# UzL-ITS/dash

Measured on AMD Instinct MI355X. Metric: online garbled inferences/sec (MiniONN CIFAR-10 CNN), higher is better.
Workload: dtype uint8 label components / int8 MFMA (exact modular arithmetic)

## Files before the change

### dash_amd/csrc/hip/mrs_chain.h

```cpp
#pragma once

#include "gadget_common.h"

namespace dash {
namespace dev {

__device__ __forceinline__ u128 add_packed(u128 a, u128 b, u128 hmask) {
    return ((a & ~hmask) + (b & ~hmask)) ^ ((a ^ b) & hmask);
}

#ifndef DASH_MRS_CHUNK
#define DASH_MRS_CHUNK 4
#endif
constexpr int kMrsChunk = DASH_MRS_CHUNK;
#ifndef DASH_MRS_M2CH
#define DASH_MRS_M2CH 16
#endif
template <int K>
__device__ __forceinline__ constexpr int mrs_pair(int l, int j) {
    return l * (2 * K - l - 1) / 2 + (j - l - 1);
}

template <int MODE>
__device__ __forceinline__ constexpr uint32_t mrs_row_sub(int i) {
    return tw_sub(MODE == 1 ? kTwSmrs : kTwMrs, static_cast<uint32_t>(i));
}
__device__ __forceinline__ void store_ypads(const MrsArgs& a, u128 key, int b, int64_t N, int64_t e) {
    const uint64_t g = a.rgate0 ^ static_cast<uint64_t>(e);
    for (int blk = 0; 4 * blk < a.ny; ++blk) {
        u128 p[4];
        hard_block(key, g, tw_sub(kTwMmy, 0), static_cast<uint32_t>(blk), p);
#pragma unroll
        for (int q = 0; q < 4; ++q)
            if (4 * blk + q < a.ny) a.ys[(static_cast<int64_t>(b) * a.ny + 4 * blk + q) * N + e] = p[q];
    }
}

template <int MODE>
__device__ __forceinline__ void store_sign_key(const MrsArgs& a, u128 key, int b, int64_t N, int64_t e) {
    if (MODE >= 1 && a.ks) a.ks[static_cast<int64_t>(b) * N + e] = key;
}

#ifndef DASH_CHAIN2_WAVES
#define DASH_CHAIN2_WAVES 4
#endif
template <int K, int MODE>
__global__ __launch_bounds__(kAesBlock, MODE == 2 ? DASH_CHAIN2_WAVES : DASH_UA_MINBLOCKS) void k_mrs_chain(MrsArgs a, Act x, const ModC* mc,
                                                                          const uint32_t* te0, const uint32_t* rk) {
    (void)te0;
    (void)rk;
    const int b = blockIdx.z;
    const int64_t N = a.N;
    constexpr int NP = K * (K - 1) / 2 > 0 ? K * (K - 1) / 2 : 1;
    for (int64_t e = static_cast<int64_t>(blockIdx.x) * blockDim.x + threadIdx.x; e < N;
         e += static_cast<int64_t>(gridDim.x) * blockDim.x) {
        const u128* row0 = a.tab + (static_cast<int64_t>(b) * N + e) * a.n_tab;
        u128* PS = a.ps + static_cast<int64_t>(b) * NP * N + e;
        u128 acc = 0;
#pragma unroll
        for (int i = 0; i < (MODE >= 1 ? K - 1 : K); ++i) {
            const int r = MODE >= 1 ? (i + 1) % K : i;
            const ModC m = mc[a.crt.p[r]];
            const int n = static_cast<int>(m.n);
            const act_t* L = x.p[r] + static_cast<int64_t>(b) * n * N + e;
            DigitStream ds[K > 1 ? K - 1 : 1];
#pragma unroll
            for (int l = 0; l < i; ++l) ds[l].init(PS[static_cast<int64_t>(mrs_pair<K>(l, i)) * N]);
            CompressFwd cf;
            cf.init();
            uint32_t col = 0;
            uint16_t cur[kMrsChunk], nxt[kMrsChunk];
#pragma unroll
            for (int u = 0; u < kMrsChunk; ++u)
                if (u < n) cur[u] = static_cast<uint16_t>(L[static_cast<int64_t>(u) * N]);
            for (int c0 = 0; c0 < n; c0 += kMrsChunk) {
#pragma unroll
                for (int u = 0; u < kMrsChunk; ++u)
                    if (c0 + kMrsChunk + u < n) nxt[u] = static_cast<uint16_t>(L[static_cast<int64_t>(c0 + kMrsChunk + u) * N]);
#pragma unroll
                for (int u = 0; u < kMrsChunk; ++u)
                    if (c0 + u < n) {
                        uint32_t d = cur[u];
#pragma unroll
                        for (int l = 0; l < i; ++l) {
                            const uint32_t s = ds[l].next(m);
                            d = d >= s ? d - s : d + m.q - s;
                        }
                        if (c0 + u == 0) col = d;
                        cf.push(d, m);
                    }
#pragma unroll
                for (int u = 0; u < kMrsChunk; ++u) cur[u] = nxt[u];
            }
            constexpr int kExtra = MODE == 1 ? 0 : 1;
            const int nt = K - 1 - i + kExtra;
            const u128* row = row0 + a.dig_off[i] + static_cast<int64_t>(col) * nt;
            u128 E[K];
#pragma unroll
            for (int t = 0; t < nt; ++t) E[t] = row[t];
            hard_unmask_n<K>(E, nt, cf.finish(), a.gate0 ^ static_cast<uint64_t>(e), mrs_row_sub<MODE>(i));
#pragma unroll
            for (int t = 0; t < K - 1 - i; ++t) PS[static_cast<int64_t>(mrs_pair<K>(i, i + 1 + t)) * N] = E[t];
            if (MODE != 1) acc = add_packed(acc, E[K - 1 - i], a.hmask);
        }
        if (MODE >= 1) {
            const ModC m = mc[a.crt.p[0]];
            const act_t* L = x.p[0] + static_cast<int64_t>(b) * m.n * N + e;
            u128 key = compress_cm<DASH_MRS_M2CH>(L, N, m);
#pragma unroll
            for (int l = 0; l < K - 1; ++l) key ^= PS[static_cast<int64_t>(mrs_pair<K>(l, K - 1)) * N];
            const uint32_t c = static_cast<uint32_t>(key) & 1u;
            u128 E = 0;
            if (MODE == 2)
                E = row0[a.dig_off[K - 1] + c] - hard_pad(key, a.gate0 ^ static_cast<uint64_t>(e), mrs_row_sub<MODE>(K - 1), 0);
            store_ypads(a, key, b, N, e);
            store_sign_key<MODE>(a, key, b, N, e);
            a.cs[static_cast<int64_t>(b) * N + e] = static_cast<uint8_t>(c);
            if (MODE == 2) acc = add_packed(acc, E, a.hmask);
        }
        if (MODE == 1) continue;
        const uint32_t col = static_cast<uint32_t>(acc) & static_cast<uint32_t>(a.T - 1);
        const u128* row = row0 + a.fin_off + static_cast<int64_t>(col) * K;
        u128 F[K];
#pragma unroll
        for (int j = 0; j < K; ++j) F[j] = row[j];
        hard_unmask<K>(F, acc, a.gate0 ^ static_cast<uint64_t>(e), mrs_row_sub<0>(K));
#pragma unroll
        for (int j = 0; j < K; ++j) a.pf[(static_cast<int64_t>(b) * K + j) * N + e] = F[j];
    }
}

constexpr int kMrsBS = 512;
constexpr int kMrsCap = 64;
#ifndef DASH_STAGE_U
#define DASH_STAGE_U 2
#endif
constexpr int kStageU = DASH_STAGE_U;
#ifndef DASH_STAGE_RD
#define DASH_STAGE_RD 4
#endif
constexpr int kStageRd = DASH_STAGE_RD;
template <int K, int MODE, int I>
__device__ __forceinline__ void chain_s_pos(const MrsArgs& a, uint64_t gate, const ModC* mc, const Act& x,
                                            uint8_t* stg, int b, int64_t N, int64_t e0, int tid, bool valid,
                                            const u128* row0, u128* PS, u128& acc) {
    constexpr int kLast = MODE >= 1 ? K - 1 : K;
    if constexpr (I < kLast) {
        constexpr int i = I;
        {
            constexpr int r = MODE >= 1 ? (i + 1) % K : i;
            const ModC m = mc[a.crt.p[r]];
            const int n = static_cast<int>(m.n);
            const act_t* L = x.p[r] + static_cast<int64_t>(b) * n * N;
            uint32_t col = 0;
            u128 key;
            constexpr int kExtra = MODE == 1 ? 0 : 1;
            constexpr int nt = K - 1 - i + kExtra;
            u128 pf0 = 0, pf1 = 0;
            if constexpr (r == 0) {
                DigitStream ds[K > 1 ? K - 1 : 1];
#pragma unroll
                for (int l = 0; l < i; ++l) ds[l].init(PS[static_cast<int64_t>(mrs_pair<K>(l, i)) * N]);
                CompressFwd cf;
                cf.init();
                for (int c0 = 0; c0 < n; c0 += kMrsCap) {
                    const int cnt = min(kMrsCap, n - c0);
                    __syncthreads();
                    lds_stage_rows<kMrsBS, kStageU>(stg, L, N, e0, c0, cnt);
                    __syncthreads();
                    for (int c = 0; c < cnt; ++c) {
                        uint32_t d = valid ? stg[c * kMrsBS + tid] : 0u;
#pragma unroll
                        for (int l = 0; l < i; ++l) {
                            const uint32_t s = ds[l].next(m);
                            d = d >= s ? d - s : d + m.q - s;
                        }
                        if (c0 + c == 0) {
                            col = d;
                            const u128* rowp = row0 + a.dig_off[i] + static_cast<int64_t>(col) * nt;
                            pf0 = rowp[0];
                            pf1 = rowp[nt - 1];
                        }
                        cf.push(d, m);
                    }
                }
                key = cf.finish();
            } else {
                u128 Q[K > 1 ? K - 1 : 1];
#pragma unroll
                for (int l = 0; l < i; ++l) Q[l] = PS[static_cast<int64_t>(mrs_pair<K>(l, i)) * N];
                u128 C = 0, PW = 1;
                const int mcn = static_cast<int>(m.c);
                const int pass = kMrsCap / mcn * mcn;
                for (int p0 = 0; p0 < n; p0 += pass) {
                    const int pcnt = min(pass, n - p0);
                    __syncthreads();
                    lds_stage_rows<kMrsBS, kStageU>(stg, L, N, e0, p0, pcnt);
                    __syncthreads();
                    for (int c0 = 0; c0 < pcnt; c0 += mcn) {
                        uint32_t rr[K > 1 ? K - 1 : 1];
#pragma unroll
                        for (int l = 0; l < i; ++l) rr[l] = divmod128(Q[l], m);
                        const int cnt = min(mcn, pcnt - c0);
                        uint32_t v = 0, pt = 1;
                        auto digit = [&](int t) -> uint32_t {
                            uint32_t d = valid ? stg[(c0 + t) * kMrsBS + tid] : 0u;
#pragma unroll
                            for (int l = 0; l < i; ++l) {
                                const uint32_t sd = chunk_digit(rr[l], m);
                                d = d >= sd ? d - sd : d + m.q - sd;
                            }
                            return d;
                        };
                        int t0 = 0;
                        if (p0 + c0 == 0) {
                            const uint32_t d = digit(0);
                            col = d;
                            const u128* rowp = row0 + a.dig_off[i] + static_cast<int64_t>(col) * nt;
                            pf0 = rowp[0];
                            pf1 = rowp[nt - 1];
                            v = d;
                            pt = m.q;
                            t0 = 1;
                        }
#pragma unroll 2
                        for (int t = t0; t < cnt; ++t) {
                            const uint32_t d = digit(t);
                            v += d * pt;
                            pt *= m.q;
                        }
                        C += PW * static_cast<u128>(v);
                        PW *= static_cast<u128>(m.D);
                    }
                }
                key = C;
            }
            const u128* row = row0 + a.dig_off[i] + static_cast<int64_t>(col) * nt;
            u128 E[K];
            E[0] = pf0;
#pragma unroll
            for (int t = 1; t < nt - 1; ++t) E[t] = row[t];
            if (nt > 1) E[nt - 1] = pf1;
            hard_unmask_n<K>(E, nt, key, gate, mrs_row_sub<MODE>(i));
            if (valid) {
#pragma unroll
                for (int t = 0; t < K - 1 - i; ++t) PS[static_cast<int64_t>(mrs_pair<K>(i, i + 1 + t)) * N] = E[t];
            }
            if constexpr (MODE != 1) acc = add_packed(acc, E[K - 1 - i], a.hmask);
        }
        chain_s_pos<K, MODE, I + 1>(a, gate, mc, x, stg, b, N, e0, tid, valid, row0, PS, acc);
    }
}

template <int K, int MODE>
__global__ __launch_bounds__(kMrsBS, MODE == 2 ? DASH_CHAIN2_WAVES : DASH_UA_MINBLOCKS) void k_mrs_chain_s(
    MrsArgs a, Act x, const ModC* mc, const uint32_t* te0, const uint32_t* rk) {
    (void)te0;
    (void)rk;
    __shared__ __attribute__((aligned(16))) uint8_t stg[kMrsCap * kMrsBS];
    const int b = blockIdx.z;
    const int64_t N = a.N;
    constexpr int NP = K * (K - 1) / 2 > 0 ? K * (K - 1) / 2 : 1;
    const int tid = static_cast<int>(threadIdx.x);
    for (int64_t e0 = static_cast<int64_t>(blockIdx.x) * kMrsBS; e0 < N; e0 += static_cast<int64_t>(gridDim.x) * kMrsBS) {
        const bool valid = e0 + tid < N;
        const int64_t e = valid ? e0 + tid : N - 1;
        const u128* row0 = a.tab + (static_cast<int64_t>(b) * N + e) * a.n_tab;
        u128* PS = a.ps + static_cast<int64_t>(b) * NP * N + e;
        u128 acc = 0;
        const uint64_t gate = a.gate0 ^ static_cast<uint64_t>(e);
        chain_s_pos<K, MODE, 0>(a, gate, mc, x, stg, b, N, e0, tid, valid, row0, PS, acc);
        if (MODE >= 1) {
            const ModC m = mc[a.crt.p[0]];
            const int n = static_cast<int>(m.n);
            const act_t* L = x.p[0] + static_cast<int64_t>(b) * n * N;
            CompressFwd cf;
            cf.init();
            u128 kb = 0;
            for (int c0 = 0; c0 < n; c0 += kMrsCap) {
                const int cnt = min(kMrsCap, n - c0);
                __syncthreads();
                lds_stage_rows<kMrsBS, kStageU>(stg, L, N, e0, c0, cnt);
                __syncthreads();
                if (m.bits == 1) {
                    for (int w0 = 0; w0 < cnt; w0 += 32) {
                        uint32_t w = 0;
#pragma unroll 8
                        for (int u = 0; u < 32; ++u)
                            if (w0 + u < cnt) w |= (valid ? static_cast<uint32_t>(stg[(w0 + u) * kMrsBS + tid]) : 0u) << u;
                        kb |= static_cast<u128>(w) << (c0 + w0);
                    }
                } else {
                    for (int c = 0; c < cnt; ++c) cf.push(valid ? stg[c * kMrsBS + tid] : 0u, m);
                }
            }
            u128 key = m.bits == 1 ? kb : cf.finish();
#pragma unroll
            for (int l = 0; l < K - 1; ++l) key ^= PS[static_cast<int64_t>(mrs_pair<K>(l, K - 1)) * N];
            const uint32_t c = static_cast<uint32_t>(key) & 1u;
            u128 E = 0;
            if (MODE == 2) E = row0[a.dig_off[K - 1] + c] - hard_pad(key, gate, mrs_row_sub<MODE>(K - 1), 0);
            if (valid) {
                store_ypads(a, key, b, N, e);
                store_sign_key<MODE>(a, key, b, N, e);
                a.cs[static_cast<int64_t>(b) * N + e] = static_cast<uint8_t>(c);
            }
            if (MODE == 2) acc = add_packed(acc, E, a.hmask);
        }
        if (MODE == 1) continue;
        const uint32_t colf = static_cast<uint32_t>(acc) & static_cast<uint32_t>(a.T - 1);
        const u128* row = row0 + a.fin_off + static_cast<int64_t>(colf) * K;
        u128 F[K];
#pragma unroll
        for (int j = 0; j < K; ++j) F[j] = row[j];
        hard_unmask<K>(F, acc, gate, mrs_row_sub<0>(K));
        if (valid) {
#pragma unroll
            for (int j = 0; j < K; ++j) a.pf[(static_cast<int64_t>(b) * K + j) * N + e] = F[j];
        }
    }
}

constexpr int kMrsWBS = 256;
constexpr int kWaveU = 8;
template <int K, int MODE, int I>
__device__ __forceinline__ void chain_w_pos(const MrsArgs& a, uint64_t gate, const ModC* mc, const uint8_t* wst,
                                            const int* roff, int tid, bool valid, const u128* row0, u128* PS,
                                            u128& acc) {
    constexpr int kLast = MODE >= 1 ? K - 1 : K;
    if constexpr (I < kLast) {
        constexpr int r = MODE >= 1 ? (I + 1) % K : I;
        const ModC m = mc[a.crt.p[r]];
        const int n = static_cast<int>(m.n);
        const uint8_t* Ls = wst + roff[r] * kMrsWBS + tid;
        uint32_t col = 0;
        u128 key;
        constexpr int kExtra = MODE == 1 ? 0 : 1;
        constexpr int nt = K - 1 - I + kExtra;
        u128 pf0 = 0, pf1 = 0;
        if constexpr (r == 0) {
            DigitStream ds[I > 0 ? I : 1];
#pragma unroll
            for (int l = 0; l < I; ++l) ds[l].init(PS[mrs_pair<K>(l, I)]);
            CompressFwd cf;
            cf.init();
            for (int c = 0; c < n; ++c) {
                uint32_t d = valid ? Ls[c * kMrsWBS] : 0u;
#pragma unroll
                for (int l = 0; l < I; ++l) {
                    const uint32_t s = ds[l].next(m);
                    d = d >= s ? d - s : d + m.q - s;
                }
                if (c == 0) {
                    col = d;
                    const u128* rowp = row0 + a.dig_off[I] + static_cast<int64_t>(col) * nt;
                    pf0 = rowp[0];
                    pf1 = rowp[nt - 1];
                }
                cf.push(d, m);
            }
            key = cf.finish();
        } else {
            u128 Q[I > 0 ? I : 1];
#pragma unroll
            for (int l = 0; l < I; ++l) Q[l] = PS[mrs_pair<K>(l, I)];
            u128 C = 0, PW = 1;
            for (int c0 = 0; c0 < n; c0 += static_cast<int>(m.c)) {
                uint32_t rr[I > 0 ? I : 1];
#pragma unroll
                for (int l = 0; l < I; ++l) rr[l] = divmod128(Q[l], m);
                const int cnt = min(static_cast<int>(m.c), n - c0);
                uint32_t v = 0, pt = 1;
                for (int t = 0; t < cnt; ++t) {
                    uint32_t d = valid ? Ls[(c0 + t) * kMrsWBS] : 0u;
#pragma unroll
                    for (int l = 0; l < I; ++l) {
                        const uint32_t sd = chunk_digit(rr[l], m);
                        d = d >= sd ? d - sd : d + m.q - sd;
                    }
                    if (c0 + t == 0) {
                        col = d;
                        const u128* rowp = row0 + a.dig_off[I] + static_cast<int64_t>(col) * nt;
                        pf0 = rowp[0];
                        pf1 = rowp[nt - 1];
                    }
                    v += d * pt;
                    pt *= m.q;
                }
                C += PW * static_cast<u128>(v);
                PW *= static_cast<u128>(m.D);
            }
            key = C;
        }
        const u128* row = row0 + a.dig_off[I] + static_cast<int64_t>(col) * nt;
        u128 E[nt > 0 ? nt : 1];
        E[0] = pf0;
#pragma unroll
        for (int t = 1; t < nt - 1; ++t) E[t] = row[t];
        if constexpr (nt > 1) E[nt - 1] = pf1;
        if constexpr (nt > 0) hard_unmask<nt>(E, key, gate, mrs_row_sub<MODE>(I));
#pragma unroll
        for (int t = 0; t < K - 1 - I; ++t) PS[mrs_pair<K>(I, I + 1 + t)] = E[t];
        if constexpr (MODE != 1) acc = add_packed(acc, E[K - 1 - I], a.hmask);
        chain_w_pos<K, MODE, I + 1>(a, gate, mc, wst, roff, tid, valid, row0, PS, acc);
    }
}

template <int K, int MODE>
__global__ __launch_bounds__(kMrsWBS, 1) void k_mrs_chain_w(MrsArgs a, Act x, const ModC* mc, const uint32_t* te0,
                                                            const uint32_t* rk) {
    (void)te0;
    (void)rk;
    extern __shared__ __attribute__((aligned(16))) uint8_t wst[];
    const int b = blockIdx.z;
    const int64_t N = a.N;
    constexpr int NP = K * (K - 1) / 2 > 0 ? K * (K - 1) / 2 : 1;
    const int tid = static_cast<int>(threadIdx.x);
    int roff[K + 1];
    const act_t* src[K];
    roff[0] = 0;
#pragma unroll
    for (int r = 0; r < K; ++r) {
        const int n = static_cast<int>(mc[a.crt.p[r]].n);
        roff[r + 1] = roff[r] + n;
        src[r] = x.p[r] + static_cast<int64_t>(b) * n * N;
    }
    const int units = roff[K] * (kMrsWBS / 16);
    for (int64_t e0 = static_cast<int64_t>(blockIdx.x) * kMrsWBS; e0 < N; e0 += static_cast<int64_t>(gridDim.x) * kMrsWBS) {
        __syncthreads();
        if (N % 16 != 0) {
            constexpr int kWaveBU = 32;
            const int bunits = roff[K] * kMrsWBS;
            const int64_t e = e0 + tid;
            for (int x0 = tid; x0 < bunits; x0 += kWaveBU * kMrsWBS) {
                uint32_t v[kWaveBU];
#pragma unroll
                for (int h = 0; h < kWaveBU; ++h) {
                    const int xu = x0 + h * kMrsWBS;
                    const int g = xu / kMrsWBS;
                    const act_t* row = src[0] + static_cast<int64_t>(g) * N;
#pragma unroll
                    for (int r = 1; r < K; ++r)
                        if (g >= roff[r]) row = src[r] + static_cast<int64_t>(g - roff[r]) * N;
                    v[h] = (xu < bunits && e < N) ? static_cast<uint32_t>(row[e]) : 0u;
                }
#pragma unroll
                for (int h = 0; h < kWaveBU; ++h) {
                    const int xu = x0 + h * kMrsWBS;
                    if (xu < bunits) wst[xu] = static_cast<uint8_t>(v[h]);
                }
            }
        } else
        for (int x0 = tid; x0 < units; x0 += kWaveU * kMrsWBS) {
            uint4 v[kWaveU];
#pragma unroll
            for (int h = 0; h < kWaveU; ++h) {
                const int xu = x0 + h * kMrsWBS;
                const int g = xu >> 4;
                const int64_t e = e0 + 16 * (xu & 15);
                const act_t* row = src[0] + static_cast<int64_t>(g) * N;
#pragma unroll
                for (int r = 1; r < K; ++r)
                    if (g >= roff[r]) row = src[r] + static_cast<int64_t>(g - roff[r]) * N;
                if (xu < units && e < N) v[h] = *reinterpret_cast<const uint4*>(row + e);
            }
#pragma unroll
            for (int h = 0; h < kWaveU; ++h) {
                const int xu = x0 + h * kMrsWBS;
                if (xu < units) *reinterpret_cast<uint4*>(wst + (xu >> 4) * kMrsWBS + 16 * (xu & 15)) = v[h];
            }
        }
        __syncthreads();
        const bool valid = e0 + tid < N;
        const int64_t e = valid ? e0 + tid : N - 1;
        const u128* row0 = a.tab + (static_cast<int64_t>(b) * N + e) * a.n_tab;
        u128 PS[NP];
        u128 acc = 0;
        const uint64_t gate = a.gate0 ^ static_cast<uint64_t>(e);
        chain_w_pos<K, MODE, 0>(a, gate, mc, wst, roff, tid, valid, row0, PS, acc);
        if (MODE >= 1) {
            const ModC m = mc[a.crt.p[0]];
            const int n = static_cast<int>(m.n);
            const uint8_t* Ls = wst + tid;
            CompressFwd cf;
            cf.init();
            for (int c = 0; c < n; ++c) cf.push(valid ? Ls[c * kMrsWBS] : 0u, m);
            u128 key = cf.finish();
#pragma unroll
            for (int l = 0; l < K - 1; ++l) key ^= PS[mrs_pair<K>(l, K - 1)];
            const uint32_t cb = static_cast<uint32_t>(key) & 1u;
            u128 E = 0;
            if (MODE == 2) E = row0[a.dig_off[K - 1] + cb] - hard_pad(key, gate, mrs_row_sub<MODE>(K - 1), 0);
            if (valid) {
                store_ypads(a, key, b, N, e);
                store_sign_key<MODE>(a, key, b, N, e);
                a.cs[static_cast<int64_t>(b) * N + e] = static_cast<uint8_t>(cb);
            }
            if (MODE == 2) acc = add_packed(acc, E, a.hmask);
        }
        if (MODE == 1) continue;
        const uint32_t colf = static_cast<uint32_t>(acc) & static_cast<uint32_t>(a.T - 1);
        const u128* row = row0 + a.fin_off + static_cast<int64_t>(colf) * K;
        u128 F[K];
#pragma unroll
        for (int j = 0; j < K; ++j) F[j] = row[j];
        hard_unmask<K>(F, acc, gate, mrs_row_sub<0>(K));
        if (valid) {
#pragma unroll
            for (int j = 0; j < K; ++j) a.pf[(static_cast<int64_t>(b) * K + j) * N + e] = F[j];
        }
    }
}

constexpr int kMrsQE = 64;
constexpr int kMrsQBS = 4 * kMrsQE;
template <int S>
__device__ __forceinline__ uint32_t quad_bcast(uint32_t v) {
    return static_cast<uint32_t>(__builtin_amdgcn_mov_dpp(static_cast<int>(v), S * 0x55, 0xF, 0xF, false));
}
template <int S>
__device__ __forceinline__ u128 quad_bcast128(u128 v) {
    const uint32_t w0 = quad_bcast<S>(static_cast<uint32_t>(v)), w1 = quad_bcast<S>(static_cast<uint32_t>(v >> 32));
    const uint32_t w2 = quad_bcast<S>(static_cast<uint32_t>(v >> 64)), w3 = quad_bcast<S>(static_cast<uint32_t>(v >> 96));
    return (static_cast<u128>((static_cast<uint64_t>(w3) << 32) | w2) << 64) | ((static_cast<uint64_t>(w1) << 32) | w0);
}
__device__ __forceinline__ uint32_t quad_sum_mod(uint32_t v, uint32_t q) {
    uint32_t s = v + static_cast<uint32_t>(__builtin_amdgcn_mov_dpp(static_cast<int>(v), 0xB1, 0xF, 0xF, false));
    s = s >= q ? s - q : s;
    uint32_t t = s + static_cast<uint32_t>(__builtin_amdgcn_mov_dpp(static_cast<int>(s), 0x4E, 0xF, 0xF, false));
    return t >= q ? t - q : t;
}
__device__ __forceinline__ uint32_t quad_sum_bytes(uint32_t v) {
    const uint32_t s = v + static_cast<uint32_t>(__builtin_amdgcn_mov_dpp(static_cast<int>(v), 0xB1, 0xF, 0xF, false));
    return s + static_cast<uint32_t>(__builtin_amdgcn_mov_dpp(static_cast<int>(s), 0x4E, 0xF, 0xF, false));
}
constexpr int kQSplit = 5;
template <int NSTR>
__device__ __forceinline__ u128 quad_key_split(const uint8_t* Ls, const ModC& m, int g, bool valid, u128 (&Q)[NSTR > 0 ? NSTR : 1]) {
    const int n = static_cast<int>(m.n);
    if (m.bits) {
        const int cpl = (n + 3) >> 2, b = static_cast<int>(m.bits);
        u128 P = 0;
        for (int t = 0; t < cpl; ++t) {
            const int idx = g * cpl + t;
            if (valid && idx < n) P |= static_cast<u128>(Ls[idx * kMrsQE]) << (b * idx);
        }
        return quad_sum128(P);
    }
    const int c = static_cast<int>(m.c);
    const uint32_t q = m.q;
    const int nch = (n + c - 1) / c;
    QPow pw;
    pw.init(m);
    u128 PW = pw.first(g), P = 0;
    for (int j = 0; 4 * j < nch; ++j) {
        uint32_t mine[NSTR > 0 ? NSTR : 1];
        if constexpr (NSTR > 0) {
#pragma unroll
            for (int l = 0; l < NSTR; ++l) mine[l] = 0;
#pragma unroll
            for (int u = 0; u < 4; ++u) {
                if (4 * j + u >= nch) break;
#pragma unroll
                for (int l = 0; l < NSTR; ++l) {
                    const uint32_t rr = divmod128(Q[l], m);
                    mine[l] = u == g ? rr : mine[l];
                }
            }
        }
        const int i = 4 * j + g;
        uint32_t v = 0, pt = 1;
        for (int t = 0; t < c; ++t) {
            const int idx = i * c + t;
            uint32_t d = 0;
            if (valid && idx < n) d = Ls[idx * kMrsQE];
            if constexpr (NSTR > 0) {
                uint32_t S = 0;
#pragma unroll
                for (int l = 0; l < NSTR; ++l) {
                    S += chunk_digit(mine[l], m);
                    S = S >= q ? S - q : S;
                }
                d = d >= S ? d - S : d + q - S;
                if (idx >= n) d = 0;
            }
            v += d * pt;
            pt *= q;
        }
        P += PW * static_cast<u128>(v);
        PW *= pw.d4;
    }
    return quad_sum128(P);
}
template <int K, int MODE, int I>
__device__ __forceinline__ void chain_q_pos(const MrsArgs& a, uint64_t gate, const ModC* mc, const uint8_t* wst,
                                            const int* roff, int el, int g, bool valid, const u128* row0, u128* PS,
                                            u128& acc) {
    constexpr int kLast = MODE >= 1 ? K - 1 : K;
    if constexpr (I < kLast) {
        constexpr int r = MODE >= 1 ? (I + 1) % K : I;
        const ModC m = mc[a.crt.p[r]];
        const int n = static_cast<int>(m.n);
        const uint8_t* Ls = wst + roff[r] * kMrsQE + el;
        constexpr int kExtra = MODE == 1 ? 0 : 1;
        constexpr int nt = K - 1 - I + kExtra;
        uint32_t col = 0;
        u128 key;
        constexpr int kNE = kQCoop ? nt : 4;
        u128 Eo[kNE];
#pragma unroll
        for (int t = 0; t < kNE; ++t) Eo[t] = 0;
        auto fetch_row = [&](uint32_t c) {
            const u128* rowp = row0 + a.dig_off[I] + static_cast<int64_t>(c) * nt;
#pragma unroll
            for (int q = 0; q < kNE; ++q)
                if (kQCoop || 4 * g + q < nt) Eo[q] = rowp[kQCoop ? q : 4 * g + q];
        };
        bool split = false;
        if constexpr (I <= kQSplit) split = I < (a.qpack >> 1);
        if (split) {
            u128 Q[I > 0 ? I : 1];
            uint32_t d0 = valid ? Ls[0] : 0u;
            if constexpr (I > 0) {
#pragma unroll
                for (int l = 0; l < I; ++l) Q[l] = PS[mrs_pair<K>(l, I)];
                uint32_t S0 = 0;
                if (m.bits) {
#pragma unroll
                    for (int l = 0; l < I; ++l) S0 += static_cast<uint32_t>(Q[l]) & (m.q - 1);
                    S0 &= m.q - 1;
                } else {
#pragma unroll
                    for (int l = 0; l < I; ++l) {
                        u128 t = Q[l];
                        uint32_t c0 = divmod128(t, m);
                        S0 += chunk_digit(c0, m);
                        S0 = S0 >= m.q ? S0 - m.q : S0;
                    }
                }
                d0 = d0 >= S0 ? d0 - S0 : d0 + m.q - S0;
            }
            col = d0;
            fetch_row(col);
            key = quad_key_split<I>(Ls, m, g, valid, Q);
        } else if constexpr (r == 0) {
            CompressFwd cf;
            cf.init();
            for (int c = 0; c < n; ++c) {
                const uint32_t d = valid ? Ls[c * kMrsQE] : 0u;
                if (c == 0) {
                    col = d;
                    fetch_row(col);
                }
                cf.push(d, m);
            }
            key = cf.finish();
        } else {
            constexpr int NS = I > 0 ? (I + 3) / 4 : 1;
            u128 Q[NS];
#pragma unroll
            for (int s2 = 0; s2 < NS; ++s2) {
                Q[s2] = 0;
#pragma unroll
                for (int l = 4 * s2; l < 4 * s2 + 4 && l < I; ++l)
                    if (g == l - 4 * s2) Q[s2] = PS[mrs_pair<K>(l, I)];
            }
            u128 C = 0, PW = 1;
            const int mcn = static_cast<int>(m.c);
            const uint32_t q = m.q;
            for (int c0 = 0; c0 < n; c0 += mcn) {
                uint32_t rr[NS];
#pragma unroll
                for (int s2 = 0; s2 < NS; ++s2) rr[s2] = I > 0 ? divmod128(Q[s2], m) : 0u;
                const int cnt = min(mcn, n - c0);
                uint32_t v = 0, pt = 1;
                if (I > 0 && (a.qpack & 1) && q <= 63) {
                    for (int t0 = 0; t0 < cnt; t0 += 4) {
                        uint32_t pk = 0;
#pragma unroll
                        for (int u = 0; u < 4; ++u) {
                            if (t0 + u >= cnt) break;
                            uint32_t sd = 0;
#pragma unroll
                            for (int s2 = 0; s2 < NS; ++s2) {
                                sd += chunk_digit(rr[s2], m);
                                sd = sd >= q ? sd - q : sd;
                            }
                            pk |= sd << (8 * u);
                        }
                        pk = quad_sum_bytes(pk);
#pragma unroll
                        for (int u = 0; u < 4; ++u) {
                            if (t0 + u >= cnt) break;
                            uint32_t S = (pk >> (8 * u)) & 0xffu;
                            S = S >= 2 * q ? S - 2 * q : S;
                            S = S >= q ? S - q : S;
                            uint32_t d = valid ? Ls[(c0 + t0 + u) * kMrsQE] : 0u;
                            d = d >= S ? d - S : d + q - S;
                            if (c0 + t0 + u == 0) {
                                col = d;
                                fetch_row(col);
                            }
                            v += d * pt;
                            pt *= q;
                        }
                    }
                } else {
                    for (int t = 0; t < cnt; ++t) {
                        uint32_t S = 0;
                        if constexpr (I > 0) {
                            uint32_t sd = 0;
#pragma unroll
                            for (int s2 = 0; s2 < NS; ++s2) {
                                sd += chunk_digit(rr[s2], m);
                                sd = sd >= q ? sd - q : sd;
                            }
                            S = quad_sum_mod(sd, q);
                        }
                        uint32_t d = valid ? Ls[(c0 + t) * kMrsQE] : 0u;
                        d = d >= S ? d - S : d + q - S;
                        if (c0 + t == 0) {
                            col = d;
                            fetch_row(col);
                        }
                        v += d * pt;
                        pt *= q;
                    }
                }
                C += PW * static_cast<u128>(v);
                PW *= static_cast<u128>(m.D);
            }
            key = C;
        }
        u128 E[nt];
        if constexpr (kQCoop) {
#pragma unroll
            for (int bk = 0; bk < (nt + 3) / 4; ++bk) {
                uint32_t w[4];
                hard_block_q(key, gate, mrs_row_sub<MODE>(I), static_cast<uint32_t>(bk), g, w);
#pragma unroll
                for (int qq = 0; qq < 4; ++qq)
                    if (4 * bk + qq < nt) E[4 * bk + qq] = Eo[4 * bk + qq] - quad_gather128(w[qq]);
            }
        } else {
            if (4 * g < nt) {
                u128 pd[4];
                hard_block(key, gate, mrs_row_sub<MODE>(I), static_cast<uint32_t>(g), pd);
#pragma unroll
                for (int qq = 0; qq < 4; ++qq)
                    if (4 * g + qq < nt) Eo[qq] -= pd[qq];
            }
#pragma unroll
            for (int t = 0; t < nt; ++t) {
                const u128 own = Eo[t % 4];
                E[t] = (t >> 2) == 0 ? quad_bcast128<0>(own) : (t >> 2) == 1 ? quad_bcast128<1>(own)
                       : (t >> 2) == 2 ? quad_bcast128<2>(own) : quad_bcast128<3>(own);
            }
        }
#pragma unroll
        for (int t = 0; t < K - 1 - I; ++t) PS[mrs_pair<K>(I, I + 1 + t)] = E[t];
        if constexpr (MODE != 1) acc = add_packed(acc, E[K - 1 - I], a.hmask);
        chain_q_pos<K, MODE, I + 1>(a, gate, mc, wst, roff, el, g, valid, row0, PS, acc);
    }
}

template <int K, int MODE>
__global__ __launch_bounds__(kMrsQBS, 2) void k_mrs_chain_q(MrsArgs a, Act x, const ModC* mc) {
    extern __shared__ __attribute__((aligned(16))) uint8_t wst[];
    const int b = blockIdx.z;
    const int64_t N = a.N;
    constexpr int NP = K * (K - 1) / 2 > 0 ? K * (K - 1) / 2 : 1;
    const int tid = static_cast<int>(threadIdx.x);
    const int el = tid >> 2, g = tid & 3;
    int roff[K + 1];
    const act_t* src[K];
    roff[0] = 0;
#pragma unroll
    for (int r = 0; r < K; ++r) {
        const int n = static_cast<int>(mc[a.crt.p[r]].n);
        roff[r + 1] = roff[r] + n;
        src[r] = x.p[r] + static_cast<int64_t>(b) * n * N;
    }
    for (int64_t e0 = static_cast<int64_t>(blockIdx.x) * kMrsQE; e0 < N; e0 += static_cast<int64_t>(gridDim.x) * kMrsQE) {
        __syncthreads();
        if (N % 16 == 0) {
            constexpr int W = kMrsQE / 16;
            const int units = roff[K] * W;
            for (int x0 = tid; x0 < units; x0 += 4 * kMrsQBS) {
                uint4 v[4];
#pragma unroll
                for (int h = 0; h < 4; ++h) {
                    const int xu = x0 + h * kMrsQBS;
                    const int gg = xu / W;
                    const int64_t e = e0 + 16 * (xu % W);
                    const act_t* row = src[0] + static_cast<int64_t>(gg) * N;
#pragma unroll
                    for (int r = 1; r < K; ++r)
                        if (gg >= roff[r]) row = src[r] + static_cast<int64_t>(gg - roff[r]) * N;
                    if (xu < units && e < N) v[h] = *reinterpret_cast<const uint4*>(row + e);
                }
#pragma unroll
                for (int h = 0; h < 4; ++h) {
                    const int xu = x0 + h * kMrsQBS;
                    if (xu < units) *reinterpret_cast<uint4*>(wst + (xu / W) * kMrsQE + 16 * (xu % W)) = v[h];
                }
            }
        } else {
            const int bunits = roff[K] * kMrsQE;
            for (int xu = tid; xu < bunits; xu += kMrsQBS) {
                const int gg = xu / kMrsQE;
                const int64_t e = e0 + xu % kMrsQE;
                const act_t* row = src[0] + static_cast<int64_t>(gg) * N;
#pragma unroll
                for (int r = 1; r < K; ++r)
                    if (gg >= roff[r]) row = src[r] + static_cast<int64_t>(gg - roff[r]) * N;
                wst[xu] = e < N ? static_cast<uint8_t>(row[e]) : 0;
            }
        }
        __syncthreads();
        const bool valid = e0 + el < N;
        const int64_t e = valid ? e0 + el : N - 1;
        const u128* row0 = a.tab + (static_cast<int64_t>(b) * N + e) * a.n_tab;
        u128 PS[NP];
        u128 acc = 0;
        const uint64_t gate = a.gate0 ^ static_cast<uint64_t>(e);
        chain_q_pos<K, MODE, 0>(a, gate, mc, wst, roff, el, g, valid, row0, PS, acc);
        if (MODE >= 1) {
            const ModC m = mc[a.crt.p[0]];
            const int n = static_cast<int>(m.n);
            const uint8_t* Ls = wst + el;
            u128 key;
            if (m.bits == 1) {
                uint32_t w = 0;
#pragma unroll 8
                for (int u = 0; u < 32; ++u) {
                    const int c = 32 * g + u;
                    if (valid && c < n) w |= static_cast<uint32_t>(Ls[c * kMrsQE]) << u;
                }
                key = quad_sum128(static_cast<u128>(w) << (32 * g));
            } else {
                CompressFwd cf;
                cf.init();
                for (int c = 0; c < n; ++c) cf.push(valid ? Ls[c * kMrsQE] : 0u, m);
                key = cf.finish();
            }
#pragma unroll
            for (int l = 0; l < K - 1; ++l) key ^= PS[mrs_pair<K>(l, K - 1)];
            const uint32_t cb = static_cast<uint32_t>(key) & 1u;
            u128 E = 0;
            if (MODE == 2) {
                if constexpr (kQCoop) {
                    uint32_t w[4];
                    hard_block_q(key, gate, mrs_row_sub<MODE>(K - 1), 0u, g, w);
                    E = row0[a.dig_off[K - 1] + cb] - quad_gather128(w[0]);
                } else {
                    E = row0[a.dig_off[K - 1] + cb] - hard_pad(key, gate, mrs_row_sub<MODE>(K - 1), 0);
                }
            }
            if (kQCoop && valid) {
                const uint64_t gy = a.rgate0 ^ static_cast<uint64_t>(e);
                for (int bk = 0; 4 * bk < a.ny; ++bk) {
                    uint32_t w[4];
                    hard_block_q(key, gy, tw_sub(kTwMmy, 0), static_cast<uint32_t>(bk), g, w);
#pragma unroll
                    for (int qq = 0; qq < 4; ++qq)
                        if (4 * bk + qq < a.ny)
                            reinterpret_cast<uint32_t*>(a.ys + (static_cast<int64_t>(b) * a.ny + 4 * bk + qq) * N + e)[g] = w[qq];
                }
                if (g == 0) a.cs[static_cast<int64_t>(b) * N + e] = static_cast<uint8_t>(cb);
            }
            if (!kQCoop && valid) {
                const uint64_t gy = a.rgate0 ^ static_cast<uint64_t>(e);
                if (4 * g < a.ny) {
                    u128 pd[4];
                    hard_block(key, gy, tw_sub(kTwMmy, 0), static_cast<uint32_t>(g), pd);
#pragma unroll
                    for (int qq = 0; qq < 4; ++qq)
                        if (4 * g + qq < a.ny) a.ys[(static_cast<int64_t>(b) * a.ny + 4 * g + qq) * N + e] = pd[qq];
                }
                if (g == 0) a.cs[static_cast<int64_t>(b) * N + e] = static_cast<uint8_t>(cb);
            }
            if (valid && g == 0) store_sign_key<MODE>(a, key, b, N, e);
            if (MODE == 2) acc = add_packed(acc, E, a.hmask);
        }
        if (MODE == 1) continue;
        const uint32_t colf = static_cast<uint32_t>(acc) & static_cast<uint32_t>(a.T - 1);
        const u128* row = row0 + a.fin_off + static_cast<int64_t>(colf) * K;
        if constexpr (kQCoop) {
#pragma unroll
            for (int bk = 0; bk < (K + 3) / 4; ++bk) {
                const bool mine = 4 * bk + g < K;
                const u128 F = mine ? row[4 * bk + g] : u128(0);
                uint32_t w[4];
                hard_block_q(acc, gate, mrs_row_sub<0>(K), static_cast<uint32_t>(bk), g, w);
                u128 pd = 0;
#pragma unroll
                for (int qq = 0; qq < 4; ++qq) {
                    const u128 p = quad_gather128(w[qq]);
                    pd = qq == g ? p : pd;
                }
                if (valid && mine) a.pf[(static_cast<int64_t>(b) * K + 4 * bk + g) * N + e] = F - pd;
            }
        } else if (4 * g < K) {
            u128 F[4], pd[4];
#pragma unroll
            for (int qq = 0; qq < 4; ++qq) F[qq] = 4 * g + qq < K ? row[4 * g + qq] : u128(0);
            hard_block(acc, gate, mrs_row_sub<0>(K), static_cast<uint32_t>(g), pd);
            if (valid) {
#pragma unroll
                for (int qq = 0; qq < 4; ++qq)
                    if (4 * g + qq < K) a.pf[(static_cast<int64_t>(b) * K + 4 * g + qq) * N + e] = F[qq] - pd[qq];
            }
        }
    }
}

static inline bool mrs_odd_base(const CrtInfo& crt) {
    if ((crt.p[0] & (crt.p[0] - 1)) != 0) return false;
    for (int r = 1; r < crt.k; ++r)
        if ((crt.p[r] & 1) == 0) return false;
    return true;
}
static inline size_t mrs_wave_lds(const MrsArgs& a, int B) {
    static const bool on = [] {
        const char* e = std::getenv("DASH_MRS_WAVE");
        return !(e && e[0] == '0');
    }();
    if (!mrs_odd_base(a.crt)) return 0;
    if (!on || (a.N % 16 != 0 && a.N > kMrsWBS) || (a.N + kMrsWBS - 1) / kMrsWBS * B > num_cus()) return 0;
    size_t sum = 0;
    for (int r = 0; r < a.crt.k; ++r) sum += static_cast<size_t>(std::floor(128.0 / std::log2(static_cast<double>(a.crt.p[r]))));
    const size_t bytes = sum * kMrsWBS;
    if (bytes > (160u << 10)) return 0;
    return bytes;
}

static inline bool mrs_quad_on() {
    static const bool on = [] {
        const char* e = std::getenv("DASH_MRS_QUAD");
        return !(e && e[0] == '0');
    }();
    return on;
}
static inline void chain_log(const char* form, int K, int mode, dim3 grid, dim3 block) {
    if (!launch_log_on()) return;
    launch_log_add(std::string("chain.") + form + " K=" + std::to_string(K) + " mode=" + std::to_string(mode), grid, block);
}
template <int K, int MODE>
static void launch_chain_w(const MrsArgs& a, const Act& x, int B, size_t wl, const ModC* mc, const AesGlobals& g,
                           hipStream_t st) {
    if (mrs_quad_on()) {
        static const int qpack = [] {
            const char* e = std::getenv("DASH_MRS_QPACK");
            const char* f = std::getenv("DASH_MRS_QSPLIT");
            const int lim = f ? std::max(-1, std::min(kQSplit, std::atoi(f))) : 3;
            return (e && e[0] == '0' ? 0 : 1) | ((lim + 1) << 1);
        }();
        MrsArgs aq = a;
        aq.qpack = qpack;
        const size_t ql = wl / kMrsWBS * kMrsQE;
        const dim3 gq(static_cast<unsigned>((a.N + kMrsQE - 1) / kMrsQE), 1, B);
        chain_log("quad", K, MODE, gq, dim3(kMrsQBS));
        hipLaunchKernelGGL((k_mrs_chain_q<K, MODE>), gq, dim3(kMrsQBS), ql, st, aq, x, mc);
        return;
    }
    static const bool raised = [] {
        return hipFuncSetAttribute(reinterpret_cast<const void*>(&k_mrs_chain_w<K, MODE>),
                                   hipFuncAttributeMaxDynamicSharedMemorySize,
                                   160 << 10) == hipSuccess;
    }();
    (void)raised;
    const dim3 gw(static_cast<unsigned>((a.N + kMrsWBS - 1) / kMrsWBS), 1, B);
    chain_log("wave", K, MODE, gw, dim3(kMrsWBS));
    hipLaunchKernelGGL((k_mrs_chain_w<K, MODE>), gw, dim3(kMrsWBS), wl, st, a, x, mc, g.te0, g.rk);
}

static inline bool mrs_staged(const MrsArgs& a, int B) {
    return mrs_odd_base(a.crt) && stage_ok(a.N, kMrsBS) && (a.N + kMrsBS - 1) / kMrsBS * B >= 2 * num_cus();
}


template <int K>
void launch_mrs_chain_k(const MrsArgs& a, const Act& x, int B, const ModC* mc, const AesGlobals& g, hipStream_t st) {
    const bool stg = mrs_staged(a, B);
    const size_t wl = stg ? 0 : mrs_wave_lds(a, B);
    const dim3 gc = stg ? grid_aes(a.N, kMrsBS, 1, B) : grid_aes(a.N, aes_bs(a.N, 1, B), 1, B);
    const dim3 bc(stg ? kMrsBS : aes_bs(a.N, 1, B));
    if (!wl) chain_log(stg ? "staged" : "lane", K, a.mode == 1 || a.mode == 2 ? a.mode : 0, gc, bc);
    if (a.mode == 1) {
        if (wl) launch_chain_w<K, 1>(a, x, B, wl, mc, g, st);
        else if (stg) hipLaunchKernelGGL((k_mrs_chain_s<K, 1>), gc, bc, 0, st, a, x, mc, g.te0, g.rk);
        else hipLaunchKernelGGL((k_mrs_chain<K, 1>), gc, bc, 0, st, a, x, mc, g.te0, g.rk);
    } else if (a.mode == 2) {
        if (wl) launch_chain_w<K, 2>(a, x, B, wl, mc, g, st);
        else if (stg) hipLaunchKernelGGL((k_mrs_chain_s<K, 2>), gc, bc, 0, st, a, x, mc, g.te0, g.rk);
        else hipLaunchKernelGGL((k_mrs_chain<K, 2>), gc, bc, 0, st, a, x, mc, g.te0, g.rk);
    } else {
        if (wl) launch_chain_w<K, 0>(a, x, B, wl, mc, g, st);
        else if (stg) hipLaunchKernelGGL((k_mrs_chain_s<K, 0>), gc, bc, 0, st, a, x, mc, g.te0, g.rk);
        else hipLaunchKernelGGL((k_mrs_chain<K, 0>), gc, bc, 0, st, a, x, mc, g.te0, g.rk);
    }
}

}
}
```

Before: 3740.

## Keep MRS chain pair values in LDS slots and fold final-pair XORs in registers

Pair values produced by one chain position and consumed by a later one are assigned at compile time to a small set of per-thread LDS slots via an interval-allocation map, with overflow pairs still spilled to the HBM scratch buffer. In sign modes, the pairs feeding the last position are XOR-folded into a register accumulator instead of being stored and reloaded. This removes global memory round-trips for intermediate digits. In exchange it raises LDS per block, which may reduce occupancy. It also switches the staging helper to a new template flag and trims the E array to its exact size.

```diff
diff --git a/dash_amd/csrc/hip/mrs_chain.h b/dash_amd/csrc/hip/mrs_chain.h
--- a/dash_amd/csrc/hip/mrs_chain.h
+++ b/dash_amd/csrc/hip/mrs_chain.h
@@ -131,7 +131,131 @@
 }
 
 constexpr int kMrsBS = 512;
-constexpr int kMrsCap = 64;
+#ifndef DASH_CHAIN_LDS_SLOTS
+#define DASH_CHAIN_LDS_SLOTS 1
+#endif
+constexpr int kChainSlots = DASH_CHAIN_LDS_SLOTS;
+#ifndef DASH_CHAIN_FOLD
+#define DASH_CHAIN_FOLD 1
+#endif
+constexpr bool kChainFold = DASH_CHAIN_FOLD != 0;
+#ifndef DASH_MRS_CAP
+#define DASH_MRS_CAP (DASH_CHAIN_LDS_SLOTS > 6 ? 32 : 64)
+#endif
+constexpr int kMrsCap = DASH_MRS_CAP;
+constexpr int kChainLds = kChainSlots * 16 * kMrsBS + kMrsCap * kMrsBS;
+static_assert(kChainSlots >= 0 && kChainSlots * 16 * kMrsBS <= (64 << 10), "slot offsets are instruction immediates (16 bits)");
+static_assert(kChainLds <= (80 << 10), "two staged-chain blocks per CU: at most 80 KiB of LDS each");
+static_assert(kMrsCap >= 20 && kMrsCap % 4 == 0, "a staging pass holds whole chunks: m.c <= 20 (p = 3)");
+
+constexpr int kPsHbm = -1;
+constexpr int kPsFold = -2;
+constexpr int kPsNone = -3;
+constexpr int chain_pair_idx(int K, int l, int j) { return l * (2 * K - l - 1) / 2 + (j - l - 1); }
+template <int K>
+struct ChainSlotMap {
+    int slot[K * (K - 1) / 2 > 0 ? K * (K - 1) / 2 : 1];
+};
+template <int K, int MODE, int S>
+constexpr ChainSlotMap<K> chain_slot_map() {
+    ChainSlotMap<K> r{};
+    constexpr int jmax = MODE >= 1 && kChainFold ? K - 2 : K - 1;
+    int live[K + 1] = {};
+    for (int l = 0; l < K; ++l)
+        for (int j = l + 1; j < K; ++j) {
+            const int p = chain_pair_idx(K, l, j);
+            if (j > jmax) r.slot[p] = kPsFold;
+            else if (S <= 0) r.slot[p] = kPsHbm;
+            else {
+                r.slot[p] = kPsNone;
+                for (int t = l; t < j; ++t) ++live[t];
+            }
+        }
+    while (true) {
+        int tp = 0;
+        for (int t = 1; t < K; ++t)
+            if (live[t] > live[tp]) tp = t;
+        if (live[tp] <= S) break;
+        int bl = -1, bj = -1;
+        for (int l = 0; l <= tp; ++l)
+            for (int j = tp + 1; j <= jmax; ++j)
+                if (r.slot[chain_pair_idx(K, l, j)] == kPsNone && (bl < 0 || j - l > bj - bl)) bl = l, bj = j;
+        r.slot[chain_pair_idx(K, bl, bj)] = kPsHbm;
+        for (int t = bl; t < bj; ++t) --live[t];
+    }
+    int busy_to[S > 0 ? S : 1] = {};
+    for (int l = 0; l < K; ++l)
+        for (int j = l + 1; j <= jmax; ++j) {
+            const int p = chain_pair_idx(K, l, j);
+            if (r.slot[p] != kPsNone) continue;
+            for (int s = 0; s < S; ++s)
+                if (busy_to[s] <= l) {
+                    r.slot[p] = s;
+                    busy_to[s] = j;
+                    break;
+                }
+        }
+    return r;
+}
+template <int K, int MODE, int S>
+constexpr bool chain_slot_map_ok() {
+    const ChainSlotMap<K> m = chain_slot_map<K, MODE, S>();
+    for (int l = 0; l < K; ++l)
+        for (int j = l + 1; j < K; ++j) {
+            const int s = m.slot[chain_pair_idx(K, l, j)];
+            if (MODE >= 1 && kChainFold && j == K - 1) {
+                if (s != kPsFold) return false;
+                continue;
+            }
+            if (s != kPsHbm && (s < 0 || s >= S)) return false;
+            if (s < 0) continue;
+            for (int l2 = 0; l2 < K; ++l2)
+                for (int j2 = l2 + 1; j2 < K; ++j2)
+                    if ((l2 != l || j2 != j) && m.slot[chain_pair_idx(K, l2, j2)] == s && l < j2 && l2 < j) return false;
+        }
+    return true;
+}
+template <int S, int... Ks>
+constexpr bool chain_slot_maps_ok() {
+    return ((chain_slot_map_ok<Ks, 0, S>() && chain_slot_map_ok<Ks, 1, S>() && chain_slot_map_ok<Ks, 2, S>()) && ...);
+}
+static_assert(chain_slot_maps_ok<kChainSlots, 2, 3, 4, 5, 6, 7, 8, 9, 10, 11, 12>(), "pair slot map (build's slot count)");
+static_assert(chain_slot_maps_ok<6, 2, 3, 4, 5, 6, 7, 8, 9, 10, 11, 12>() && chain_slot_maps_ok<8, 2, 3, 4, 5, 6, 7, 8, 9, 10, 11, 12>() &&
+                  chain_slot_maps_ok<1, 2, 3, 4, 5, 6, 7, 8, 9, 10, 11, 12>() && chain_slot_maps_ok<0, 2, 3, 4, 5, 6, 7, 8, 9, 10, 11, 12>(),
+              "pair slot map (the measured slot counts, one slot, none)");
+static_assert(!kChainFold ||
+                  (chain_slot_map<7, 2, 6>().slot[chain_pair_idx(7, 0, 4)] == kPsHbm && chain_slot_map<7, 2, 6>().slot[chain_pair_idx(7, 0, 5)] == kPsHbm &&
+                   chain_slot_map<7, 2, 6>().slot[chain_pair_idx(7, 1, 5)] == kPsHbm && chain_slot_map<7, 2, 6>().slot[chain_pair_idx(7, 0, 3)] >= 0),
+              "K = 7 joint chain: the three longest-lived pairs overflow");
+template <int K, int MODE>
+struct ChainSlotsOf {
+    static constexpr ChainSlotMap<K> map = chain_slot_map<K, MODE, kChainSlots>();
+};
+template <int K, int MODE, int I, int T = 0, int NT>
+__device__ __forceinline__ void chain_s_put(const u128 (&E)[NT], u128* PS, u128* psl, int64_t N, bool valid, u128& sx) {
+    if constexpr (T < K - 1 - I) {
+        constexpr int p = chain_pair_idx(K, I, I + 1 + T);
+        constexpr int s = ChainSlotsOf<K, MODE>::map.slot[p];
+        if constexpr (s == kPsFold) {
+            uint64_t lo = static_cast<uint64_t>(sx ^ E[T]), hi = static_cast<uint64_t>((sx ^ E[T]) >> 64);
+            asm("" : "+v"(lo), "+v"(hi));
+            sx = (static_cast<u128>(hi) << 64) | lo;
+        } else if constexpr (s >= 0) psl[s * kMrsBS] = E[T];
+        else if (valid) PS[static_cast<int64_t>(p) * N] = E[T];
+        chain_s_put<K, MODE, I, T + 1>(E, PS, psl, N, valid, sx);
+    }
+}
+template <int K, int MODE, int I, bool LDS, int L = 0, int NQ>
+__device__ __forceinline__ void chain_s_get(u128 (&Q)[NQ], const u128* PS, const u128* psl, int64_t N) {
+    if constexpr (L < I) {
+        constexpr int p = chain_pair_idx(K, L, I);
+        constexpr int s = ChainSlotsOf<K, MODE>::map.slot[p];
+        static_assert(s != kPsFold && s != kPsNone, "a folded pair has no reader");
+        if constexpr (LDS && s >= 0) Q[L] = psl[s * kMrsBS];
+        if constexpr (!LDS && s < 0) Q[L] = PS[static_cast<int64_t>(p) * N];
+        chain_s_get<K, MODE, I, LDS, L + 1>(Q, PS, psl, N);
+    }
+}
 #ifndef DASH_STAGE_U
 #define DASH_STAGE_U 2
 #endif
@@ -143,8 +267,9 @@
 template <int K, int MODE, int I>
 __device__ __forceinline__ void chain_s_pos(const MrsArgs& a, uint64_t gate, const ModC* mc, const Act& x,
                                             uint8_t* stg, int b, int64_t N, int64_t e0, int tid, bool valid,
-                                            const u128* row0, u128* PS, u128& acc) {
+                                            const u128* row0, u128* PS, u128* psl, u128& acc, u128& sx) {
     constexpr int kLast = MODE >= 1 ? K - 1 : K;
+    constexpr int NQ = I > 0 ? I : 1;
     if constexpr (I < kLast) {
         constexpr int i = I;
         {
@@ -158,15 +283,18 @@
             constexpr int nt = K - 1 - i + kExtra;
             u128 pf0 = 0, pf1 = 0;
             if constexpr (r == 0) {
-                DigitStream ds[K > 1 ? K - 1 : 1];
-#pragma unroll
-                for (int l = 0; l < i; ++l) ds[l].init(PS[static_cast<int64_t>(mrs_pair<K>(l, i)) * N]);
+                u128 Q[NQ];
+                chain_s_get<K, MODE, I, false>(Q, PS, psl, N);
+                chain_s_get<K, MODE, I, true>(Q, PS, psl, N);
+                DigitStream ds[NQ];
+#pragma unroll
+                for (int l = 0; l < i; ++l) ds[l].init(Q[l]);
                 CompressFwd cf;
                 cf.init();
                 for (int c0 = 0; c0 < n; c0 += kMrsCap) {
                     const int cnt = min(kMrsCap, n - c0);
                     __syncthreads();
-                    lds_stage_rows<kMrsBS, kStageU>(stg, L, N, e0, c0, cnt);
+                    lds_stage_rows<kMrsBS, kStageU, true>(stg, L, N, e0, c0, cnt);
                     __syncthreads();
                     for (int c = 0; c < cnt; ++c) {
                         uint32_t d = valid ? stg[c * kMrsBS + tid] : 0u;
@@ -186,19 +314,19 @@
                 }
                 key = cf.finish();
             } else {
-                u128 Q[K > 1 ? K - 1 : 1];
-#pragma unroll
-                for (int l = 0; l < i; ++l) Q[l] = PS[static_cast<int64_t>(mrs_pair<K>(l, i)) * N];
+                u128 Q[NQ];
+                chain_s_get<K, MODE, I, false>(Q, PS, psl, N);
                 u128 C = 0, PW = 1;
                 const int mcn = static_cast<int>(m.c);
                 const int pass = kMrsCap / mcn * mcn;
                 for (int p0 = 0; p0 < n; p0 += pass) {
                     const int pcnt = min(pass, n - p0);
                     __syncthreads();
-                    lds_stage_rows<kMrsBS, kStageU>(stg, L, N, e0, p0, pcnt);
+                    lds_stage_rows<kMrsBS, kStageU, true>(stg, L, N, e0, p0, pcnt);
                     __syncthreads();
+                    if (p0 == 0) chain_s_get<K, MODE, I, true>(Q, PS, psl, N);
                     for (int c0 = 0; c0 < pcnt; c0 += mcn) {
-                        uint32_t rr[K > 1 ? K - 1 : 1];
+                        uint32_t rr[NQ];
 #pragma unroll
                         for (int l = 0; l < i; ++l) rr[l] = divmod128(Q[l], m);
                         const int cnt = min(mcn, pcnt - c0);
@@ -236,19 +364,16 @@
                 key = C;
             }
             const u128* row = row0 + a.dig_off[i] + static_cast<int64_t>(col) * nt;
-            u128 E[K];
+            u128 E[nt];
             E[0] = pf0;
 #pragma unroll
             for (int t = 1; t < nt - 1; ++t) E[t] = row[t];
-            if (nt > 1) E[nt - 1] = pf1;
-            hard_unmask_n<K>(E, nt, key, gate, mrs_row_sub<MODE>(i));
-            if (valid) {
-#pragma unroll
-                for (int t = 0; t < K - 1 - i; ++t) PS[static_cast<int64_t>(mrs_pair<K>(i, i + 1 + t)) * N] = E[t];
-            }
+            if constexpr (nt > 1) E[nt - 1] = pf1;
+            hard_unmask<nt>(E, key, gate, mrs_row_sub<MODE>(i));
+            chain_s_put<K, MODE, I>(E, PS, psl, N, valid, sx);
             if constexpr (MODE != 1) acc = add_packed(acc, E[K - 1 - i], a.hmask);
         }
-        chain_s_pos<K, MODE, I + 1>(a, gate, mc, x, stg, b, N, e0, tid, valid, row0, PS, acc);
+        chain_s_pos<K, MODE, I + 1>(a, gate, mc, x, stg, b, N, e0, tid, valid, row0, PS, psl, acc, sx);
     }
 }
 
@@ -257,19 +382,22 @@
     MrsArgs a, Act x, const ModC* mc, const uint32_t* te0, const uint32_t* rk) {
     (void)te0;
     (void)rk;
-    __shared__ __attribute__((aligned(16))) uint8_t stg[kMrsCap * kMrsBS];
+    __shared__ __attribute__((aligned(16))) uint8_t lds[kChainLds];
     const int b = blockIdx.z;
     const int64_t N = a.N;
     constexpr int NP = K * (K - 1) / 2 > 0 ? K * (K - 1) / 2 : 1;
     const int tid = static_cast<int>(threadIdx.x);
+    u128* psl = reinterpret_cast<u128*>(lds) + tid;
+    uint8_t* stg = lds + kChainSlots * 16 * kMrsBS;
     for (int64_t e0 = static_cast<int64_t>(blockIdx.x) * kMrsBS; e0 < N; e0 += static_cast<int64_t>(gridDim.x) * kMrsBS) {
         const bool valid = e0 + tid < N;
         const int64_t e = valid ? e0 + tid : N - 1;
         const u128* row0 = a.tab + (static_cast<int64_t>(b) * N + e) * a.n_tab;
         u128* PS = a.ps + static_cast<int64_t>(b) * NP * N + e;
         u128 acc = 0;
+        u128 sx = 0;
         const uint64_t gate = a.gate0 ^ static_cast<uint64_t>(e);
-        chain_s_pos<K, MODE, 0>(a, gate, mc, x, stg, b, N, e0, tid, valid, row0, PS, acc);
+        chain_s_pos<K, MODE, 0>(a, gate, mc, x, stg, b, N, e0, tid, valid, row0, PS, psl, acc, sx);
         if (MODE >= 1) {
             const ModC m = mc[a.crt.p[0]];
             const int n = static_cast<int>(m.n);
@@ -280,7 +408,7 @@
             for (int c0 = 0; c0 < n; c0 += kMrsCap) {
                 const int cnt = min(kMrsCap, n - c0);
                 __syncthreads();
-                lds_stage_rows<kMrsBS, kStageU>(stg, L, N, e0, c0, cnt);
+                lds_stage_rows<kMrsBS, kStageU, true>(stg, L, N, e0, c0, cnt);
                 __syncthreads();
                 if (m.bits == 1) {
                     for (int w0 = 0; w0 < cnt; w0 += 32) {
@@ -295,8 +423,15 @@
                 }
             }
             u128 key = m.bits == 1 ? kb : cf.finish();
-#pragma unroll
-            for (int l = 0; l < K - 1; ++l) key ^= PS[static_cast<int64_t>(mrs_pair<K>(l, K - 1)) * N];
+            if constexpr (kChainFold) {
+                key ^= sx;
+            } else {
+                u128 Q[K > 1 ? K - 1 : 1];
+                chain_s_get<K, MODE, K - 1, false>(Q, PS, psl, N);
+                chain_s_get<K, MODE, K - 1, true>(Q, PS, psl, N);
+#pragma unroll
+                for (int l = 0; l < K - 1; ++l) key ^= Q[l];
+            }
             const uint32_t c = static_cast<uint32_t>(key) & 1u;
             u128 E = 0;
             if (MODE == 2) E = row0[a.dig_off[K - 1] + c] - hard_pad(key, gate, mrs_row_sub<MODE>(K - 1), 0);
```

After: 3934, median of 6. +5.2%, better.
